# OPTML-Group/Unlearn-Saliency

Hardware: AMD Instinct MI355X
Metric: unlearn_steps_per_sec (ResNet-18/CIFAR-10 10%-forget, RL + SalUn mask, batch 256/GPU) (higher is better)
Workload: dtype f32

## Files before the change

### include/salun.h

```cpp
#ifndef SALUN_H
#define SALUN_H

#include <stddef.h>
#include <stdint.h>

#ifdef __cplusplus
extern "C" {
#endif

#define SALUN_OK 0
#define SALUN_EINVAL (-22)
#define SALUN_ENOSPC (-28)
#define SALUN_EIO (-5)

#define SALUN_MAX_THRESHOLDS 16

typedef void *salun_stream_t;

int salun_version(void);
const char *salun_strerror(int code);
const char *salun_arch(void);
int salun_clock_probe(unsigned long long *out , int samples, int spins, salun_stream_t stream);

int salun_saliency_accumulate(float *acc , const float *g ,
// ... 64 lines not shown
                     void *ws , size_t ws_bytes, salun_stream_t stream);

int salun_fim_square_accumulate(float *F , float *tmp , double n_data,
                                int64_t n, salun_stream_t stream);

int salun_conv2d_forward(const float *x , const float *w , const float *bias ,
                         float *y , int N, int C, int H, int W, int K, int R, int stride, int pad,
                         int P, int Q, salun_stream_t stream);
int salun_conv2d_forward_fused(const float *x , const float *w , const float *bias ,
                               const float *nbias , const float *addend ,
                               float *y , int N, int C, int H, int W, int K, int R, int stride, int pad,
                               int P, int Q, void *ws , size_t ws_bytes, salun_stream_t stream);
size_t salun_conv2d_data_workspace_bytes(int N, int outC, int outH, int outW, int R, int conv_stride);
int salun_conv2d_backward_data_ws(const float *dy , const float *w , const float *addend ,
                                  float *dx , int N, int C, int H, int W, int K, int R, int stride, int pad,
                                  int P, int Q, void *ws , size_t ws_bytes, salun_stream_t stream);
int salun_conv2d_backward_data(const float *dy , const float *w , float *dx , int N, int C,
                               int H, int W, int K, int R, int stride, int pad, int P, int Q,
                               salun_stream_t stream);
int salun_conv2d_backward_data_add(const float *dy , const float *w , const float *addend ,
                                   float *dx , int N, int C, int H, int W, int K, int R, int stride, int pad,
                                   int P, int Q, salun_stream_t stream);
size_t salun_channel_sum_workspace_bytes(int N, int K);
int salun_channel_sum(const float *dy , float *out , int N, int K, int HW, int accumulate,
                      void *ws , size_t ws_bytes, salun_stream_t stream);
size_t salun_conv2d_wgrad_workspace_bytes(int N, int C, int K, int R, int P, int Q);
int salun_conv2d_backward_weight(const float *x , const float *dy , float *dw , int N, int C,
                                 int H, int W, int K, int R, int stride, int pad, int P, int Q, int accumulate,
                                 void *ws , size_t ws_bytes, salun_stream_t stream);
#define SALUN_WGRAD_SHARED 1u
int salun_conv2d_backward_weight_ex(const float *x , const float *dy , float *dw , int N, int C,
                                    int H, int W, int K, int R, int stride, int pad, int P, int Q, int accumulate,
                                    unsigned flags, void *ws , size_t ws_bytes, salun_stream_t stream);
#define SALUN_ROUTE_FORWARD 0
#define SALUN_ROUTE_BACKWARD_DATA 1
#define SALUN_ROUTE_BACKWARD_WEIGHT 2
#define SALUN_ROUTE_EPI 2u
#define SALUN_ROUTE_W_UNALIGNED 4u
#define SALUN_ROUTE_OUT_UNALIGNED 8u
#define SALUN_ROUTE_IN_UNALIGNED 16u
int salun_conv2d_route(int direction, int N, int C, int H, int W, int K, int R, int stride, int pad, int P, int Q,
                       unsigned flags, size_t ws_bytes, char *buf, size_t buflen, int *nsplit );

size_t salun_conv3x3_pack_bytes(int K, int C, int dgrad);
#define SALUN_PACK_MAX_JOBS 32
typedef struct {
  const float *w;
  float *img_fwd;
  float *img_dgrad;
  int32_t K, C;
} salun_pack_job_t;
int salun_conv3x3_pack_weights(const salun_pack_job_t *jobs , int njobs, salun_stream_t stream);
int salun_conv3x3_packed(const float *x , const float *img , const float *bias ,
                         const float *nbias , const float *addend , float *y ,
                         int N, int Cred, int H, int W, int Kout, int cfg, salun_stream_t stream);

int salun_conv2d_bf16_supported(int C, int K, int R, int stride, int pad);
int salun_conv2d_bf16_pack_weights(const float *w , uint16_t *wp , int K, int C, int R,
                                   salun_stream_t stream);
#define SALUN_BF16_PACK_MAX_JOBS 64
typedef struct {
  const float *w;
  uint16_t *wp;
  int32_t K, C, R, transposed;
} salun_bf16_pack_job_t;
int salun_bf16_pack_weights_batch(const salun_bf16_pack_job_t *jobs, int n, salun_stream_t stream);
// ... 248 lines not shown
```

### unlearn_saliency_amd/_lib.py

```python
from __future__ import annotations

import ctypes
import os
import subprocess

_HERE = os.path.dirname(os.path.abspath(__file__))
LIB_PATH = os.environ.get("SALUN_LIB") or os.path.join(_HERE, "libsalun.so")
CSRC_DIR = os.path.join(_HERE, "csrc")

SALUN_OK = 0
SALUN_EINVAL = -22
SALUN_ENOSPC = -28
SALUN_EIO = -5
SALUN_MAX_THRESHOLDS = 16
SALUN_TOPK_FORCE_FULL_SCAN = 1
SALUN_TOPK_VALUES_ONLY = 2
SALUN_WGRAD_SHARED = 1

c_void_p, c_int, c_int64, c_uint64 = ctypes.c_void_p, ctypes.c_int, ctypes.c_int64, ctypes.c_uint64
c_double, c_size_t = ctypes.c_double, ctypes.c_size_t

class GemmSeg(ctypes.Structure):
    _fields_ = [("A", c_void_p), ("B", c_void_p), ("K", ctypes.c_int32), ("a_i", ctypes.c_int32),
                ("a_k", ctypes.c_int32), ("b_j", ctypes.c_int32), ("b_k", ctypes.c_int32)]
# ... 52 lines not shown
                                       c_double, c_double, c_double, c_double, c_double, c_double, c_int, c_int64,
                                       c_void_p]),
    "salun_adam_coefficients": (c_int, [c_void_p, c_double, c_double, c_double, c_void_p, c_void_p]),
    "salun_masked_adam_step_coef": (c_int, [c_void_p, c_void_p, c_void_p, c_void_p, c_void_p, c_void_p, c_double,
                                            c_double, c_void_p, c_double, c_double, c_double, c_double, c_int64,
                                            c_void_p]),
    "salun_adam_ema_step": (c_int, [c_void_p, c_void_p, c_void_p, c_void_p, c_void_p, c_void_p, c_void_p, c_double,
                                    c_double, c_double, c_double, c_double, c_double, c_double, c_double, c_int, c_int64,
                                    c_void_p]),
    "salun_adam_ema_step_coef": (c_int, [c_void_p, c_void_p, c_void_p, c_void_p, c_void_p, c_void_p, c_void_p, c_double,
                                         c_double, c_void_p, c_double, c_double, c_double, c_double, c_double, c_int64,
                                         c_void_p]),
    "salun_qsample": (c_int, [c_void_p, c_void_p, c_void_p, c_void_p, c_void_p, c_int64, c_void_p, c_int64, c_int64,
                              c_void_p]),
    "salun_sqerr_workspace_bytes": (c_size_t, [c_int64, c_int64]),
    "salun_sqerr_loss": (c_int, [c_void_p, c_void_p, c_int64, c_int64, c_double, c_void_p, c_void_p, c_void_p,
                                 c_void_p, c_size_t, c_void_p]),
    "salun_fim_square_accumulate": (c_int, [c_void_p, c_void_p, c_double, c_int64, c_void_p]),
    "salun_conv2d_forward": (c_int, [c_void_p, c_void_p, c_void_p, c_void_p] + [c_int] * 10 + [c_void_p]),
    "salun_conv2d_forward_fused": (c_int, [c_void_p] * 6 + [c_int] * 10 + [c_void_p, c_size_t, c_void_p]),
    "salun_conv2d_data_workspace_bytes": (c_size_t, [c_int] * 6),
    "salun_conv2d_backward_data_ws": (c_int, [c_void_p] * 4 + [c_int] * 10 + [c_void_p, c_size_t, c_void_p]),
    "salun_conv2d_backward_data": (c_int, [c_void_p, c_void_p, c_void_p] + [c_int] * 10 + [c_void_p]),
    "salun_channel_sum_workspace_bytes": (c_size_t, [c_int] * 2),
    "salun_channel_sum": (c_int, [c_void_p, c_void_p] + [c_int] * 4 + [c_void_p, c_size_t, c_void_p]),
    "salun_conv2d_wgrad_workspace_bytes": (c_size_t, [c_int] * 6),
    "salun_conv3x3_pack_bytes": (c_size_t, [c_int] * 3),
    "salun_conv3x3_pack_weights": (c_int, [c_void_p, c_int, c_void_p]),
    "salun_conv3x3_packed": (c_int, [c_void_p] * 6 + [c_int] * 6 + [c_void_p]),
    "salun_conv2d_backward_weight": (c_int, [c_void_p, c_void_p, c_void_p] + [c_int] * 11 + [c_void_p, c_size_t,
                                                                                          c_void_p]),
    "salun_conv2d_backward_weight_ex": (c_int, [c_void_p, c_void_p, c_void_p] + [c_int] * 11 + [ctypes.c_uint, c_void_p,
                                                                                                 c_size_t, c_void_p]),
    "salun_conv2d_route": (c_int, [c_int] * 11 + [ctypes.c_uint, c_size_t, ctypes.c_char_p, c_size_t,
                                   ctypes.POINTER(c_int)]),
    "salun_conv2d_bf16_supported": (c_int, [c_int] * 5),
    "salun_conv2d_bf16_pack_weights": (c_int, [c_void_p, c_void_p, c_int, c_int, c_int, c_void_p]),
    "salun_bf16_pack_weights_batch": (c_int, [c_void_p, c_int, c_void_p]),
    "salun_conv2d_bf16_data_workspace_bytes": (c_size_t, [c_int] * 8),
    "salun_conv2d_bf16_forward": (c_int, [c_void_p] * 6 + [c_int] * 8 + [c_void_p, c_size_t, c_void_p]),
    "salun_conv2d_bf16_backward_data": (c_int, [c_void_p] * 4 + [c_int] * 8 + [c_void_p, c_size_t, c_void_p]),
    "salun_conv2d_bf16_wgrad_workspace_bytes": (c_size_t, [c_int] * 8),
    "salun_conv2d_bf16_backward_weight": (c_int, [c_void_p] * 4 + [c_int] * 9 + [c_void_p, c_size_t, c_void_p]),
    "salun_colsum_bf16_workspace_bytes": (c_size_t, [c_int]),
    "salun_colsum_bf16": (c_int, [c_void_p, c_void_p, c_void_p, c_int64, c_int, c_int, c_int, c_void_p, c_size_t, c_void_p]),
    "salun_conv2d_bf16_backward_weight_ex": (c_int, [c_void_p] * 5 + [c_int] * 9 + [c_void_p, c_size_t, c_void_p]),
    "salun_gn_bf16_workspace_bytes": (c_size_t, [c_int] * 4),
    "salun_gn_bf16_forward": (c_int, [c_void_p] * 6 + [c_int] * 4 + [c_double, c_int, c_void_p, c_size_t, c_void_p]),
    "salun_gn_bf16_backward": (c_int, [c_void_p] * 8 + [c_int] * 6 + [c_void_p, c_size_t, c_void_p]),
    "salun_attn_supported": (c_int, [c_int]),
    "salun_attn_forward": (c_int, [c_void_p] * 5 + [c_int] * 5 + [ctypes.c_longlong, c_int] * 4 + [c_double, c_void_p]),
    "salun_attn_backward": (c_int, [c_void_p] * 10 + [c_int] * 5 + [ctypes.c_longlong, c_int] * 5 + [c_double, c_void_p]),
    "salun_ln_bf16_workspace_bytes": (c_size_t, [c_int64, c_int]),
    "salun_ln_bf16_forward": (c_int, [c_void_p] * 5 + [c_int64, c_int, c_double, c_void_p]),
    "salun_ln_bf16_backward": (c_int, [c_void_p] * 7 + [c_int64, c_int, c_int, c_void_p, c_size_t, c_void_p]),
    "salun_geglu_bf16_forward": (c_int, [c_void_p, c_void_p, c_int64, c_int, c_void_p]),
    "salun_geglu_bf16_backward": (c_int, [c_void_p, c_void_p, c_void_p, c_int64, c_int, c_void_p]),
    "salun_bn_workspace_bytes": (c_size_t, [c_int]),
    "salun_bn_forward": (c_int, [c_void_p] * 10 + [c_int] * 4 + [c_double, c_double, c_int, c_void_p, c_size_t, c_void_p]),
    "salun_bn_backward": (c_int, [c_void_p] * 12 + [c_int] * 5 + [c_void_p, c_size_t, c_void_p]),
    "salun_conv2d_backward_data_add": (c_int, [c_void_p] * 4 + [c_int] * 10 + [c_void_p]),
    "salun_gn_workspace_bytes": (c_size_t, [c_int, c_int]),
    "salun_gn_forward": (c_int, [c_void_p] * 6 + [c_int] * 4 + [c_double, c_int, c_void_p]),
    "salun_gn_backward": (c_int, [c_void_p] * 11 + [c_int] * 5 + [c_void_p, c_size_t, c_void_p]),
    "salun_gn_backward_fused": (c_int, [c_void_p] * 15 + [c_int] * 5 + [c_void_p, c_size_t, c_void_p]),
    "salun_param_diff": (c_int, [c_void_p, c_void_p, c_void_p, c_int64, c_void_p]),
# ... 102 lines not shown
```

### unlearn_saliency_amd/csrc/salun_conv.hip

```cpp
#include "salun_common.h"
#include "salun_conv_plan.h"
#include <mutex>
#include <type_traits>
#include <unordered_set>

int salun_ring_wgrad_launch(const float *x, const float *dy, float *part, int N, int C, int H, int W, int K, int nsplit,
                            int nchunks, hipStream_t st);

namespace {

typedef float f32x16 __attribute__((ext_vector_type(16)));

struct PatchPos {
  int goff;
  int loff;
  int valid;
};

__device__ __forceinline__ void tile_origin(int tile, int NI, int TP, int tiles_per_img, int &n0, int &p0) {
  if (NI > 1) { n0 = tile * NI; p0 = 0; }
  else { n0 = tile / tiles_per_img; p0 = (tile - n0 * tiles_per_img) * TP; }
}

struct LanePix {
// ... 392 lines not shown
#pragma unroll
      for (int t = 0; t < KT; ++t) a_cur[t] = a_nxt[t];
    }
  }

  const int n_out = n0 + lp.ni;
  const int h_out = (p0 + lp.p) * g.os + g.ph, w_out = lp.q * g.os + g.pw;
  if (n_out < g.N) {
#pragma unroll
    for (int t = 0; t < KT; ++t) {
      const int kbase = k0 + (wk * KT + t) * 32 + 4 * hi;
      const size_t obase = (((size_t)n_out * g.yC + kbase) * g.yH + h_out) * g.yW + w_out;
      const size_t kstride = (size_t)g.yH * g.yW;
      float bv[16];
      const int klast = g.yC - 1 - kbase;
      if (g.bias) {
#pragma unroll
        for (int v = 0; v < 16; ++v)
          bv[v] = g.bias[obase + (long long)acc_row_clamped(v, klast, kbase) * (long long)kstride];
      }
#pragma unroll
      for (int v = 0; v < 16; ++v) {
        const int kr = acc_row(v);
        if (kbase + kr < g.yC) {
          float o = acc[t][v];
          if (g.bias) o += bv[v];
          g.y[obase + kr * kstride] = o;
        }
      }
    }
  }
}

template <int R, int PAD, int KT, int WP, int WK>
__global__ __launch_bounds__(256, 2) void conv_dgrad_s2(const float *__restrict__ dy, const float *__restrict__ w,
                                                     const float *__restrict__ addend, float *__restrict__ dx, int N,
                                                     int K, int P, int Q, int C, int H, int W, int NI, int TP,
                                                     int IH_t, int IW_t, int logQ) {
  constexpr int RS = R * R;
  constexpr int KB = WK * KT * 32;
  constexpr int WROW = CC * RS + 1;
  constexpr int DMIN = (R == 1) ? 0 : (PAD == 1 ? 0 : -1);
  constexpr int FP = (R == 1) ? 1 : 2;
  constexpr int NCLS = (R == 1) ? 1 : 4;
  extern __shared__ __attribute__((aligned(16))) float lds[];
  const int PSZ = NI * IH_t * IW_t;
  const int ch_stride = PSZ | 1;
  float *patch = lds;
  float *wl = lds + CC * ch_stride;

  const int tid = threadIdx.x, lane = tid & 63, wave = tid >> 6;
  const int lo = lane & 31, hi = lane >> 5;
  const int wp = wave % WP, wk = wave / WP;
  const int c0out = blockIdx.y * KB;
  const int tiles_per_img = (NI > 1) ? 1 : P / TP;
  const int tile = blockIdx.x;
  int n0, p0;
  if (NI > 1) { n0 = tile * NI; p0 = 0; }
  else { n0 = tile / tiles_per_img; p0 = (tile - n0 * tiles_per_img) * TP; }
  const LanePix lp = lane_pixel(wp * 32 + lo, Q, logQ, TP, IH_t, IW_t, 1);

  const int planePQ = P * Q;
  int goff = 0;
  bool valid = false;
  if (tid < PSZ) {
    const int ni = tid / (IH_t * IW_t);
    const int rem = tid - ni * (IH_t * IW_t);
    const int ih = rem / IW_t, iw = rem - ih * IW_t;
    const int n = n0 + ni;
    const int pp = p0 + DMIN + ih, qq = DMIN + iw;
    valid = (n < N) && pp >= 0 && pp < P && qq >= 0 && qq < Q;
// ... 72 lines not shown
#pragma unroll
        for (int rs = 0; rs < RS; ++rs) av[t][rs] = wb0[t * 32 * WROW + cc * RS + rs];
    };
    float b_cur[FP * FP], a_cur[KT][RS], b_nxt[FP * FP], a_nxt[KT][RS];
    operands(0, b_cur, a_cur);
#pragma unroll
    for (int step = 0; step < NSTEP; ++step) {
      if (step + 1 < NSTEP) operands(step + 1, b_nxt, a_nxt);
      __builtin_amdgcn_sched_barrier(0);
#pragma unroll
      for (int r = 0; r < R; ++r)
#pragma unroll
        for (int s2 = 0; s2 < R; ++s2) {
          const int ph = (R == 1) ? 0 : ((r - PAD) & 1), pw = (R == 1) ? 0 : ((s2 - PAD) & 1);
          const int di = (R == 1) ? 0 : ((ph + PAD - r) / 2 - DMIN), dj = (R == 1) ? 0 : ((pw + PAD - s2) / 2 - DMIN);
          const int cls = (R == 1) ? 0 : (ph * 2 + pw);
#pragma unroll
          for (int t = 0; t < KT; ++t)
            acc[cls][t] = __builtin_amdgcn_mfma_f32_32x32x2f32(a_cur[t][r * R + s2], b_cur[di * FP + dj], acc[cls][t],
                                                               0, 0, 0);
        }
      __builtin_amdgcn_sched_barrier(0);
      if (step + 1 < NSTEP) {
#pragma unroll
        for (int i = 0; i < FP * FP; ++i) b_cur[i] = b_nxt[i];
#pragma unroll
        for (int t = 0; t < KT; ++t)
#pragma unroll
          for (int rs = 0; rs < RS; ++rs) a_cur[t][rs] = a_nxt[t][rs];
      }
    }
  }

  const int n_out = n0 + lp.ni;
  const int a_out = p0 + lp.p;
  if (n_out < N) {
#pragma unroll
    for (int t = 0; t < KT; ++t) {
      const int cbase = c0out + (wk * KT + t) * 32 + 4 * hi;
      const size_t obase = (((size_t)n_out * C + cbase) * H + 2 * a_out) * W + 2 * lp.q;
      const size_t cstride = (size_t)H * W;
#pragma unroll
      for (int vb = 0; vb < 16; vb += 8) {
        float2 ad[8][2];
        const int clast = C - 1 - cbase;
        if (addend) {
#pragma unroll
          for (int u = 0; u < 8; ++u) {
            const int v = vb + u, cr = acc_row_clamped(v, clast, cbase);
#pragma unroll
            for (int ph = 0; ph < 2; ++ph)
              ad[u][ph] = *reinterpret_cast<const float2 *>(addend + obase + (long long)cr * (long long)cstride + ph * W);
          }
        }
#pragma unroll
        for (int u = 0; u < 8; ++u) {
          const int v = vb + u, cr = acc_row(v);
          if (cbase + cr < C) {
#pragma unroll
            for (int ph = 0; ph < 2; ++ph) {
              float2 o;
              if (R == 1) {
                o.x = (ph == 0) ? acc[0][t][v] : 0.f;
                o.y = 0.f;
              } else {
                o.x = acc[ph * 2 + 0][t][v];
                o.y = acc[ph * 2 + 1][t][v];
              }
              if (addend) {
                o.x += ad[u][ph].x;
                o.y += ad[u][ph].y;
              }
              *reinterpret_cast<float2 *>(dx + obase + cr * cstride + ph * W) = o;
// ... 821 lines not shown
      if (!p.fast) {
        launch_one_igemm<R, STRIDE, KT, WP, WK, DGRAD, false, 1, false, false>(p, a, st);
      } else if (p.S > 1) {
        if constexpr (CAN_SPLIT) launch_one_igemm<R, STRIDE, KT, WP, WK, DGRAD, true, 1, true, false>(p, a, st);
      } else if (p.epi) {
        if constexpr (CAN_EPI) launch_one_igemm<R, STRIDE, KT, WP, WK, DGRAD, true, 1, false, true>(p, a, st);
      } else {
        launch_one_igemm<R, STRIDE, KT, WP, WK, DGRAD, true, 1, false, false>(p, a, st);
      }
    });
  }
  SALUN_LAUNCH_CHECK();
  if (p.S > 1) {
    hipLaunchKernelGGL(conv_split_finish, dim3((unsigned)((p.out_elems / 4 + 255) / 256)), dim3(256), 0, st, a.part, p.S,
                       p.out_elems, DGRAD ? nullptr : a.bias, a.nbias, a.addend, DGRAD ? a.bias : nullptr, a.y, a.yC,
                       a.yH * a.yW);
    SALUN_LAUNCH_CHECK();
  }
  return SALUN_OK;
}

inline int launch_data(const DataPlan &p, const DataArgs &a, hipStream_t st) {
  if (p.dgrad) return p.R == 3 ? launch_data<3, 1, true>(p, a, st) : launch_data<1, 1, true>(p, a, st);
  if (p.R == 3) return p.stride == 1 ? launch_data<3, 1, false>(p, a, st) : launch_data<3, 2, false>(p, a, st);
  return p.stride == 1 ? launch_data<1, 1, false>(p, a, st) : launch_data<1, 2, false>(p, a, st);
}

template <int R, int PAD, int KT, int WP, int WK>
void launch_one_dgrad_s2(const Dgrad2Plan &p, const float *dy, const float *w, const float *addend, float *dx, int N,
                         int C, int H, int W, int K, int P, int Q, hipStream_t st) {
  const TileGeom &g = p.t.g;
  allow_lds(conv_dgrad_s2<R, PAD, KT, WP, WK>, p.lds_bytes);
  hipLaunchKernelGGL((conv_dgrad_s2<R, PAD, KT, WP, WK>), dim3(g.ntiles, C / p.t.kb()), dim3(256), p.lds_bytes, st, dy, w,
                     addend, dx, N, K, P, Q, C, H, W, g.NI, g.TP, g.IH_t, g.IW_t, g.logQ);
}

template <int RH, int RW, int KT, int WP, int WK, int MAXPOS>
void launch_one_dgrad_tap(const TapClass &c, const TapArgs &a, hipStream_t st) {
  allow_lds(conv_dgrad_tap<RH, RW, KT, WP, WK, MAXPOS>, c.lds_bytes);
  hipLaunchKernelGGL((conv_dgrad_tap<RH, RW, KT, WP, WK, MAXPOS>), dim3(c.t.g.ntiles, (a.yC + c.t.kb() - 1) / c.t.kb()),
                     dim3(256), c.lds_bytes, st, a);
}

inline int launch_dgrad_s2(const Dgrad2Plan &p, const float *dy, const float *w, const float *addend, float *dx, int N,
                           int C, int H, int W, int K, int P, int Q, hipStream_t st) {
  if (p.merged) {
    with_tile(p.t, [&](auto kt, auto wp, auto wk) {
      constexpr int KT = decltype(kt)::value, WP = decltype(wp)::value, WK = decltype(wk)::value;
      if constexpr (KT <= 2) {
        if (p.R == 1) launch_one_dgrad_s2<1, 0, KT, WP, WK>(p, dy, w, addend, dx, N, C, H, W, K, P, Q, st);
        else if (p.pad == 1) launch_one_dgrad_s2<3, 1, KT, WP, WK>(p, dy, w, addend, dx, N, C, H, W, K, P, Q, st);
        else launch_one_dgrad_s2<3, 0, KT, WP, WK>(p, dy, w, addend, dx, N, C, H, W, K, P, Q, st);
      }
    });
    SALUN_LAUNCH_CHECK();
    return SALUN_OK;
  }
  TapArgs a{};
  a.x = dy; a.w = w; a.bias = addend; a.y = dx;
  a.N = N; a.xC = K; a.xH = P; a.xW = Q; a.yC = C; a.yH = H; a.yW = W;
  a.wC = C; a.wK = K; a.Rfull = p.R;
  a.subH = H / 2; a.subW = W / 2; a.os = 2; a.ts = 2;
  if (p.any_empty) {
    const size_t bytes = sizeof(float) * (size_t)N * C * H * W;
    if (!addend) {
      if (hipMemsetAsync(dx, 0, bytes, st) != hipSuccess) return SALUN_EIO;
    } else if (addend != dx) {
// ... 225 lines not shown
  if (!dy || !out || !ws || N < 1 || K < 1 || HW < 1) return SALUN_EINVAL;
  const int S = channel_sum_splits(N, K);
  if (ws_bytes < sizeof(float) * (size_t)K * S) return SALUN_ENOSPC;
  if (K > 65535 * 16) return SALUN_EINVAL;
  hipStream_t st = salun_hip_stream(stream);
  float *part = static_cast<float *>(ws);
  hipLaunchKernelGGL(k_channel_sum_partial, dim3(K, S), dim3(256), 0, st, dy, part, N, K, HW, S);
  SALUN_LAUNCH_CHECK();
  hipLaunchKernelGGL(k_channel_sum_final, dim3((K + 255) / 256), dim3(256), 0, st, part, out, K, S, accumulate);
  SALUN_LAUNCH_CHECK();
  return SALUN_OK;
}

SALUN_EXPORT int salun_conv2d_backward_weight(const float *x, const float *dy, float *dw, int N, int C, int H, int W,
                                              int K, int R, int stride, int pad, int P, int Q, int accumulate,
                                              void *ws, size_t ws_bytes, salun_stream_t stream) {
  return salun_conv2d_backward_weight_ex(x, dy, dw, N, C, H, W, K, R, stride, pad, P, Q, accumulate, 0, ws, ws_bytes, stream);
}

SALUN_EXPORT int salun_conv2d_backward_weight_ex(const float *x, const float *dy, float *dw, int N, int C, int H, int W,
                                                 int K, int R, int stride, int pad, int P, int Q, int accumulate,
                                                 unsigned flags, void *ws, size_t ws_bytes, salun_stream_t stream) {
  if (!x || !dy || !dw || !ws) return SALUN_EINVAL;
  const WgradPlan p = plan_wgrad(N, C, H, W, K, R, stride, pad, P, Q, (flags & SALUN_WGRAD_SHARED) != 0,
                                 salun_aligned16(x) && salun_aligned16(dy), ws_bytes);
  if (p.rc != SALUN_OK) return p.rc;
  hipStream_t st = salun_hip_stream(stream);
  const WgradArgs a{x, dy, static_cast<float *>(ws), N, C, H, W, K, P, Q, pad};
  const int rc = launch_wgrad(p, a, st);
  if (rc != SALUN_OK) return rc;
  launch_wgrad_reduce(a.part, dw, (int64_t)K * C * R * R, p.nsplit, accumulate, K * C, R * R, st);
  SALUN_LAUNCH_CHECK();
  return SALUN_OK;
}

SALUN_EXPORT int salun_conv2d_route(int direction, int N, int C, int H, int W, int K, int R, int stride, int pad, int P,
                                    int Q, unsigned flags, size_t ws_bytes, char *buf, size_t buflen, int *nsplit) {
  if (!buf || buflen < 1) return SALUN_EINVAL;
  buf[0] = 0;
  if (nsplit) *nsplit = 0;
  const bool w_al16 = !(flags & SALUN_ROUTE_W_UNALIGNED), out_al16 = !(flags & SALUN_ROUTE_OUT_UNALIGNED);
  const bool in_al16 = !(flags & SALUN_ROUTE_IN_UNALIGNED);
  int rc = SALUN_EINVAL, len = 0;
  if (direction == SALUN_ROUTE_FORWARD) {
    const DataPlan p = plan_data(N, C, K, P, Q, R, stride, false, C, (flags & SALUN_ROUTE_EPI) != 0, w_al16, out_al16,
                                 ws_bytes);
    if ((rc = p.rc) == SALUN_OK) len = data_label(buf, buflen, p);
  } else if (direction == SALUN_ROUTE_BACKWARD_DATA && (P < 1 || Q < 1)) {
  } else if (direction == SALUN_ROUTE_BACKWARD_DATA && stride == 1) {
    const DataPlan p = plan_data(N, K, C, H, W, R, 1, true, C, false, w_al16, out_al16, ws_bytes);
    if ((rc = p.rc) == SALUN_OK) len = data_label(buf, buflen, p);
  } else if (direction == SALUN_ROUTE_BACKWARD_DATA && stride == 2) {
    const Dgrad2Plan p = plan_dgrad_s2(N, C, H, W, K, R, pad, P, Q, w_al16, out_al16);
    if ((rc = p.rc) == SALUN_OK) len = dgrad2_label(buf, buflen, p);
  } else if (direction == SALUN_ROUTE_BACKWARD_WEIGHT) {
    const WgradPlan p = plan_wgrad(N, C, H, W, K, R, stride, pad, P, Q, (flags & SALUN_WGRAD_SHARED) != 0, in_al16,
                                   ws_bytes);
    if ((rc = p.rc) == SALUN_OK) {
      len = wgrad_label(buf, buflen, p);
      if (nsplit) *nsplit = p.nsplit;
    }
  }
  if (rc == SALUN_OK && (len < 0 || (size_t)len >= buflen)) { buf[0] = 0; return SALUN_ENOSPC; }
  return rc;
}
```

### unlearn_saliency_amd/csrc/salun_conv_plan.h

```cpp
#pragma once
#include <cstddef>
#include <cstdio>
#include "../../include/salun.h"

bool salun_ring_wgrad_fits(int N, int C, int H, int W, int K, int nchunks, bool in_al16);

namespace {

constexpr int CC = 8;
constexpr int igemm_chunk(int R, int stride) { return (R == 1 && stride == 1) ? 32 : CC; }

constexpr int tap_chunk(int taps) { return taps == 1 ? 32 : taps == 2 ? 16 : 8; }

struct TileGeom {
  int NI, TP, IH_t, IW_t, logQ;
  int ntiles;
  bool ok;
  int psz() const { return NI * IH_t * IW_t; }
};

inline int ilog2(int v) {
  int l = 0;
  while ((1 << l) < v) ++l;
  return l;
// ... 295 lines not shown
  if (!shifts) return p;
  p.lds_bytes = sizeof(float) * 2 * ((size_t)64 * (g.psz() | 1) + (size_t)64 * (pixc + 1) + 256);
  if ((size_t)g.NI * C * H * W >= (1u << 30) || (size_t)g.NI * K * P * Q >= (1u << 30)) return p;
  if (p.lds_bytes > 160 * 1024) return p;
  p.rc = SALUN_OK;
  p.fullC = C % 64 == 0;
  if (R == 3 && stride == 1 && pad == 1 && P == H && Q == W && !shared &&
      salun_ring_wgrad_fits(N, C, H, W, K, g.ntiles, in_al16)) {
    p.route = WG_RING;
    return p;
  }
  if (R == 3 && pad == 1 && p.fullC && W % 4 == 0 && Q * stride == W && P * stride == H && in_al16 &&
      (size_t)g.NI * C * H * W < (1u << 30)) {
    const int F4C = g.NI * g.IH_t * (W / 4);
    const int nit = (F4C % 4 == 0) ? F4C / 4 : 0;
    if (stride == 1 ? (nit == 5 || nit == 6 || nit == 8) : (nit == 9 || nit == 10)) {
      p.route = WG_V;
      p.nit = nit;
    }
  }
  return p;
}

inline int wgrad_label(char *buf, size_t n, const WgradPlan &p) {
  switch (p.route) {
    case WG_1X1: return snprintf(buf, n, "wgrad_1x1<%d>", p.stride);
    case WG_SMALLC: return snprintf(buf, n, "wgrad_smallc<%d,%d>", p.R, p.stride);
    case WG_RING: return snprintf(buf, n, "wgrad_ring<W%d>", p.W);
    case WG_V: return snprintf(buf, n, "wgrad_v<%d,%d>", p.stride, p.nit);
    default: return snprintf(buf, n, "wgrad<%d,%d,%s>", p.R, p.stride, p.fullC ? "true" : "false");
  }
}

}
```

### unlearn_saliency_amd/ops.py

```python
from __future__ import annotations

import ctypes
from typing import Optional, Sequence

import torch

from .fastfn import FastFunction

from . import _lib, ringpack, weightimg
from ._lib import c_double, c_int, c_int64, c_size_t, c_uint64, c_void_p, check
from .streams import _stream, _stream_handle


def _dev(t: Optional[torch.Tensor], dtype: torch.dtype, name: str, allow_none: bool = False) -> c_void_p:
    if t is None:
        if allow_none:
            return c_void_p(None)
        raise ValueError(f"{name} must not be None")
    if not t.is_cuda:
        raise RuntimeError(f"{name}: the SalUn HIP kernels need a device tensor (got {t.device}); no CPU fallback")
    if t.dtype != dtype:
        raise TypeError(f"{name}: expected {dtype}, got {t.dtype}")
    if not t.is_contiguous():
        raise ValueError(f"{name} must be contiguous")
# ... 384 lines not shown
        return None
    check(rc, "salun_conv2d_backward_data")
    return dx


WGRAD_KERNEL = [None]


def conv2d_backward_weight(x: torch.Tensor, dy: torch.Tensor, w_shape, stride: int, pad: int,
                           out: Optional[torch.Tensor] = None, accumulate: bool = False,
                           shared: bool = False, stream: Optional[torch.cuda.Stream] = None) -> Optional[torch.Tensor]:
    N, C, H, W = x.shape
    K, _, R, _ = w_shape
    P, Q = dy.shape[2], dy.shape[3]
    L = _lib.lib()
    nbytes = L.salun_conv2d_wgrad_workspace_bytes(N, C, K, R, P, Q)
    if nbytes == 0:
        return None
    ws = workspace(nbytes, x.device, stream=stream)
    dw = out if out is not None else torch.empty(tuple(w_shape), dtype=torch.float32, device=x.device)
    rc = L.salun_conv2d_backward_weight_ex(_dev(x, torch.float32, "x"), _dev(dy, torch.float32, "dy"),
                                           _dev(dw, torch.float32, "dw"), N, C, H, W, K, R, stride, pad, P, Q,
                                           int(bool(accumulate and out is not None)),
                                           _lib.SALUN_WGRAD_SHARED if (shared if WGRAD_KERNEL[0] is None
                                                                       else WGRAD_KERNEL[0] == "shared") else 0,
                                           c_void_p(ws.data_ptr()), c_size_t(ws.numel()),
                                           c_void_p(_stream_handle() if stream is None else stream.cuda_stream))
    if rc == _lib.SALUN_EINVAL:
        return None
    check(rc, "salun_conv2d_backward_weight")
    return dw


def conv3x3_pack(w: torch.Tensor, dgrad: bool, out: Optional[torch.Tensor] = None) -> Optional[torch.Tensor]:
    K, C = w.shape[0], w.shape[1]
    L = _lib.lib()
    nbytes = int(L.salun_conv3x3_pack_bytes(K, C, int(dgrad)))
    if nbytes == 0 or tuple(w.shape[2:]) != (3, 3):
        return None
    img = out if out is not None and out.numel() * 4 == nbytes else torch.empty(nbytes // 4, dtype=torch.float32,
                                                                                device=w.device)
    _dev(w, torch.float32, "w")
    job = _lib.PackJob(w.data_ptr(), None if dgrad else img.data_ptr(), img.data_ptr() if dgrad else None, K, C)
    check(L.salun_conv3x3_pack_weights(ctypes.cast(ctypes.pointer(job), c_void_p), 1, _stream()),
          "salun_conv3x3_pack_weights")
    return img


def conv3x3_packed(x: torch.Tensor, img: torch.Tensor, Kout: int, bias: Optional[torch.Tensor] = None,
                   nbias: Optional[torch.Tensor] = None, addend: Optional[torch.Tensor] = None,
                   out: Optional[torch.Tensor] = None, cfg: int = 0) -> Optional[torch.Tensor]:
    N, Cred, H, W = x.shape
    y = out if out is not None else torch.empty((N, Kout, H, W), dtype=torch.float32, device=x.device)
    rc = _lib.lib().salun_conv3x3_packed(_dev(x, torch.float32, "x"), c_void_p(img.data_ptr()),
                                         _dev(bias, torch.float32, "bias", True),
                                         _dev(nbias, torch.float32, "nbias", True),
                                         _dev(addend, torch.float32, "addend", True), c_void_p(y.data_ptr()),
                                         N, Cred, H, W, Kout, int(cfg), _stream())
    if rc == _lib.SALUN_EINVAL:
        return None
    check(rc, "salun_conv3x3_packed")
    return y


def channel_sum(dy: torch.Tensor, out: Optional[torch.Tensor] = None, accumulate: bool = False) -> torch.Tensor:
    N, K = dy.shape[0], dy.shape[1]
# ... 527 lines not shown
```

### unlearn_saliency_amd/resblock.py

```python
from __future__ import annotations

import torch

from .fastfn import FastFunction
import torch.nn as nn

import os

from . import dist as sdist
from . import draws, gradsink, ops, wgrad_side

FWD_SHORTCUT_BESIDE = os.environ.get("SALUN_FWD_SHORTCUT_BESIDE", "1") != "0"


def _bn_args(bn: nn.BatchNorm2d):
    return bn.running_mean, bn.running_var, bn.training, bn.momentum, bn.eps


class _BasicBlockFn(FastFunction):
    @staticmethod
    def forward(ctx, x, blk, w1, g1, b1, w2, g2, b2, wd, gd, bd):
        s = blk.conv1.stride[0]
        N, C, H, W = x.shape
        P, Q = (H + 2 - 3) // s + 1, (W + 2 - 3) // s + 1
        training = blk.bn1.training
        cd = md = idd = None
        fork = None
        if wd is not None:
            def shortcut():
                cd_ = ops.conv2d_forward(x, wd, None, s, 0, P, Q)
                return (cd_,) + tuple(ops.bn_forward(cd_, None, gd, bd, *_bn_args(blk.downsample[1]), False,
                                                     blk.downsample[1].num_batches_tracked))
            if (FWD_SHORTCUT_BESIDE and wgrad_side.OVERLAP and x.is_cuda
                    and not torch.cuda.is_current_stream_capturing()):
                main, fork = torch.cuda.current_stream(x.device), wgrad_side.stream(x.device)
                fork.wait_stream(main)
                with torch.cuda.stream(fork):
                    cd, skip, md, idd = shortcut()
                x.record_stream(fork)
        c1 = ops.conv2d_forward(x, w1, None, s, 1, P, Q)
        y1, m1, i1 = ops.bn_forward(c1, None, g1, b1, *_bn_args(blk.bn1), True, blk.bn1.num_batches_tracked)
        c2 = ops.conv2d_forward(y1, w2, None, 1, 1, P, Q)
        if wd is None:
            skip = x
        elif fork is None:
            cd, skip, md, idd = shortcut()
        else:
            main.wait_stream(fork)
            for t in (cd, skip, md, idd):
                if t is not None:
                    t.record_stream(main)
        out, m2, i2 = ops.bn_forward(c2, skip, g2, b2, *_bn_args(blk.bn2), True, blk.bn2.num_batches_tracked)
        ctx.save_for_backward(x, c1, y1, c2, out, cd, w1, g1, b1, w2, g2, b2, wd, gd, bd, m1, i1, m2, i2, md, idd)
        ctx.cfg = (s, training)
        return out

    @staticmethod
    def backward(ctx, dout):
        x, c1, y1, c2, out, cd, w1, g1, b1, w2, g2, b2, wd, gd, bd, m1, i1, m2, i2, md, idd = ctx.saved_tensors
        s, training = ctx.cfg
        dout = dout.contiguous()
        grads = {}

        def bn_bwd(dy, y, xin, g, b, m, i, relu, want_dres):
            gw, gb = gradsink.sink(g), gradsink.sink(b)
            if gw is None or gb is None:
                gw = gb = None
            dx, dres, dg, db = ops.bn_backward(dy, y, xin, g, m, i, training, relu, want_dres, gw, gb)
            if gw is not None:
                gradsink.arrived(g)
                gradsink.arrived(b)
                dg = db = None
            return dx, dres, dg, db

        dev = dout.device
        overlap = wgrad_side.OVERLAP

        def wgrad(xin, dy, w, stride, pad):
            dst = gradsink.sink(w)
            if overlap:
                dw = wgrad_side.beside(dev, (xin, dy), lambda side: ops.conv2d_backward_weight(
                    xin, dy, w.shape, stride, pad, out=dst, accumulate=True, shared=True, stream=side), alloc=dst is None)
            else:
                dw = ops.conv2d_backward_weight(xin, dy, w.shape, stride, pad, out=dst, accumulate=True)
            if dst is not None:
                gradsink.arrived(w)
                return None
            return dw

        dc2, dskip, dg2, db2 = bn_bwd(dout, out, c2, g2, b2, m2, i2, True, True)
        dwd = dgd = dbd = None
        dxd = dskip
        if wd is not None:
            dcd, _, dgd, dbd = bn_bwd(dskip, None, cd, gd, bd, md, idd, False, False)
            dwd = wgrad(x, dcd, wd, s, 0)
            dxd = ops.conv2d_backward_data(dcd, wd, x.shape, s, 0) if ctx.needs_input_grad[0] else None
        dw2 = wgrad(y1, dc2, w2, 1, 1)
        dy1 = ops.conv2d_backward_data(dc2, w2, y1.shape, 1, 1)
        dc1, _, dg1, db1 = bn_bwd(dy1, y1, c1, g1, b1, m1, i1, True, False)
        dw1 = wgrad(x, dc1, w1, s, 1)
        dx = ops.conv2d_backward_data(dc1, w1, x.shape, s, 1, addend=dxd) if ctx.needs_input_grad[0] else None
        if overlap and not all(g is None for g in (dw1, dw2, dwd)):
            torch.cuda.current_stream(dev).wait_stream(wgrad_side.stream(dev))
            wgrad_side.release_held(dev)
        return dx, None, dw1, dg1, db1, dw2, dg2, db2, dwd, dgd, dbd


def _probe(blk, shape, device) -> bool:
    N, C, H, W = shape
    s = blk.conv1.stride[0]
    P, Q = (H + 2 - 3) // s + 1, (W + 2 - 3) // s + 1
    K = blk.conv1.out_channels
    if (P * Q) % 4 or (H * W) % 4:
        return False
    e = lambda *sh: torch.empty(sh, dtype=torch.float32, device=device)
    x, y1, dy = e(N, C, H, W), e(N, K, P, Q), e(N, K, P, Q)
    convs = [(x, blk.conv1.weight, s, 1), (y1, blk.conv2.weight, 1, 1)]
    if blk.downsample is not None:
        convs.append((x, blk.downsample[0].weight, s, 0))
    for xin, w, st, pad in convs:
        if ops.conv2d_forward(xin, w, None, st, pad, P, Q) is None:
            return False
        if ops.conv2d_backward_data(dy, w, xin.shape, st, pad, addend=xin) is None:
            return False
        if ops.conv2d_backward_weight(xin, dy, w.shape, st, pad) is None:
            return False
    return True


def _structure_ok(blk) -> bool:
    convs = [blk.conv1, blk.conv2] + ([blk.downsample[0]] if blk.downsample is not None else [])
    bns = [blk.bn1, blk.bn2] + ([blk.downsample[1]] if blk.downsample is not None else [])
    if any(type(b) is not nn.BatchNorm2d or not b.affine or not b.track_running_stats or b.momentum is None
           for b in bns):
        return False
    if any(c.bias is not None or c.groups != 1 or c.dilation != (1, 1) or c.weight.dtype != torch.float32
           for c in convs):
        return False
    if len({b.training for b in bns}) != 1:
        return False
    c1, c2 = blk.conv1, blk.conv2
    ok = (c1.kernel_size == (3, 3) and c1.padding == (1, 1) and c1.stride[0] == c1.stride[1] and c1.stride[0] in (1, 2)
          and c2.kernel_size == (3, 3) and c2.padding == (1, 1) and c2.stride == (1, 1))
    if blk.downsample is not None:
        d = blk.downsample[0]
        ok = ok and d.kernel_size == (1, 1) and d.padding == (0, 0) and d.stride == c1.stride
    else:
        ok = ok and c1.stride == (1, 1) and c1.in_channels == c1.out_channels
    return ok


def fused_basic_block(blk, x: torch.Tensor):
    if not (x.is_cuda and x.dtype == torch.float32 and x.dim() == 4) or torch.is_autocast_enabled():
        return None
    cache = blk.__dict__.setdefault("_fused_shapes", {})
    key = (tuple(x.shape), x.device)
    ok = cache.get(key)
    if ok is None:
        with torch.no_grad():
            ok = cache[key] = _structure_ok(blk) and _probe(blk, tuple(x.shape), x.device)
# ... 179 lines not shown
```

Baseline: 118.1.

## Fuse strided block's 3x3 and 1x1 projection data-gradients into one kernel

Adds a paired variant of the stride-2 dgrad kernel. It runs the 1x1 projection shortcut's data-gradient GEMM on the same output tile after the 3x3 conv1 dgrad and sums the two in registers before writing dx. The separate shortcut dgrad launch is dropped, along with the full-size intermediate dxd tensor and its read back as an addend. This costs extra register pressure and LDS reuse in the kernel, plus a per-shape probe cache in Python.

Measured after the change: 118.3 (median of 2 runs). No clear change (+0.1%).

```diff
diff --git a/include/salun.h b/include/salun.h
--- a/include/salun.h
+++ b/include/salun.h
@@ -120,6 +120,10 @@
 int salun_conv2d_backward_weight_ex(const float *x , const float *dy , float *dw , int N, int C,
                                     int H, int W, int K, int R, int stride, int pad, int P, int Q, int accumulate,
                                     unsigned flags, void *ws , size_t ws_bytes, salun_stream_t stream);
+int salun_conv2d_backward_data_pair(const float *dy , const float *w , const float *dy2 ,
+                                    const float *w2 , const float *addend , float *dx ,
+                                    int N, int C, int H, int W, int K, int K2, int pad, int P, int Q,
+                                    salun_stream_t stream);
 #define SALUN_ROUTE_FORWARD 0
 #define SALUN_ROUTE_BACKWARD_DATA 1
 #define SALUN_ROUTE_BACKWARD_WEIGHT 2
diff --git a/unlearn_saliency_amd/_lib.py b/unlearn_saliency_amd/_lib.py
--- a/unlearn_saliency_amd/_lib.py
+++ b/unlearn_saliency_amd/_lib.py
@@ -108,6 +108,7 @@
                                                                                           c_void_p]),
     "salun_conv2d_backward_weight_ex": (c_int, [c_void_p, c_void_p, c_void_p] + [c_int] * 11 + [ctypes.c_uint, c_void_p,
                                                                                                  c_size_t, c_void_p]),
+    "salun_conv2d_backward_data_pair": (c_int, [c_void_p] * 6 + [c_int] * 9 + [c_void_p]),
     "salun_conv2d_route": (c_int, [c_int] * 11 + [ctypes.c_uint, c_size_t, ctypes.c_char_p, c_size_t,
                                    ctypes.POINTER(c_int)]),
     "salun_conv2d_bf16_supported": (c_int, [c_int] * 5),
diff --git a/unlearn_saliency_amd/csrc/salun_conv.hip b/unlearn_saliency_amd/csrc/salun_conv.hip
--- a/unlearn_saliency_amd/csrc/salun_conv.hip
+++ b/unlearn_saliency_amd/csrc/salun_conv.hip
@@ -448,11 +448,13 @@
   }
 }
 
-template <int R, int PAD, int KT, int WP, int WK>
+template <int R, int PAD, int KT, int WP, int WK, bool PAIR = false>
 __global__ __launch_bounds__(256, 2) void conv_dgrad_s2(const float *__restrict__ dy, const float *__restrict__ w,
+                                                     const float *__restrict__ dy2, const float *__restrict__ w2,
                                                      const float *__restrict__ addend, float *__restrict__ dx, int N,
-                                                     int K, int P, int Q, int C, int H, int W, int NI, int TP,
+                                                     int K, int K2, int P, int Q, int C, int H, int W, int NI, int TP,
                                                      int IH_t, int IW_t, int logQ) {
+  static_assert(!PAIR || (R == 3 && PAD == 1), "the pair is conv1 of a strided block with its projection");
   constexpr int RS = R * R;
   constexpr int KB = WK * KT * 32;
   constexpr int WROW = CC * RS + 1;
@@ -591,13 +593,81 @@
     }
   }
 
-  const int n_out = n0 + lp.ni;
-  const int a_out = p0 + lp.p;
+  LanePix lpe = lp;
+  int hie = hi, wke = wk;
+  if constexpr (PAIR) {
+    constexpr int W2ROW = CC + 1;
+    constexpr int N2F4 = CC * KB / 4;
+    static_assert(N2F4 <= 256 && KB * W2ROW <= KB * WROW, "one 16-byte load per thread; inside the 3x3 slab's region");
+    int tid2 = threadIdx.x;
+    asm volatile("" : "+v"(tid2));
+    const int lo2 = tid2 & 31, hi2 = (tid2 >> 5) & 1, wave2 = tid2 >> 6;
+    const LanePix lp2 = lane_pixel((wave2 % WP) * 32 + lo2, Q, logQ, TP, IH_t, IW_t, 1);
+    const int goff2 = goff + (goff / planePQ / K) * (K2 - K) * planePQ;
+    const int row2 = tid2 / (KB / 4), q42 = tid2 - row2 * (KB / 4);
+    auto load_chunk2 = [&](int k0) {
+      if (valid) {
+        const float *src = dy2 + goff2 + k0 * planePQ;
+#pragma unroll
+        for (int c = 0; c < CC; ++c) preg[c] = src[c * planePQ];
+      } else {
+#pragma unroll
+        for (int c = 0; c < CC; ++c) preg[c] = 0.f;
+      }
+      if (N2F4 == 256 || tid2 < N2F4)
+        wreg4[0] = *reinterpret_cast<const float4 *>(w2 + (size_t)(k0 + row2) * C + c0out + 4 * q42);
+    };
+    auto store_chunk2 = [&]() {
+      if (tid2 < PSZ) {
+#pragma unroll
+        for (int c = 0; c < CC; ++c) patch[c * ch_stride + tid2] = preg[c];
+      }
+      if (N2F4 == 256 || tid2 < N2F4) {
+        wl[(4 * q42 + 0) * W2ROW + row2] = wreg4[0].x;
+        wl[(4 * q42 + 1) * W2ROW + row2] = wreg4[0].y;
+        wl[(4 * q42 + 2) * W2ROW + row2] = wreg4[0].z;
+        wl[(4 * q42 + 3) * W2ROW + row2] = wreg4[0].w;
+      }
+    };
+    f32x16 acc2[KT];
+#pragma unroll
+    for (int t = 0; t < KT; ++t)
+#pragma unroll
+      for (int v = 0; v < 16; ++v) acc2[t][v] = 0.f;
+    load_chunk2(0);
+    for (int k0 = 0; k0 < K2; k0 += CC) {
+      __syncthreads();
+      store_chunk2();
+      __syncthreads();
+      if (k0 + CC < K2) load_chunk2(k0 + CC);
+      const float *pb0 = patch + hi2 * ch_stride + lp2.off;
+      const float *wb0 = wl + ((wave2 / WP) * KT * 32 + lo2) * W2ROW + hi2;
+#pragma unroll
+      for (int step = 0; step < CC / 2; ++step) {
+        const float b = pb0[2 * step * ch_stride];
+#pragma unroll
+        for (int t = 0; t < KT; ++t)
+          acc2[t] = __builtin_amdgcn_mfma_f32_32x32x2f32(wb0[t * 32 * W2ROW + 2 * step], b, acc2[t], 0, 0, 0);
+      }
+    }
+#pragma unroll
+    for (int cl = 0; cl < NCLS; ++cl)
+#pragma unroll
+      for (int t = 0; t < KT; ++t)
+#pragma unroll
+        for (int v = 0; v < 16; ++v) acc[cl][t][v] += (cl == 0) ? acc2[t][v] : 0.f;
+    lpe = lp2;
+    hie = hi2;
+    wke = wave2 / WP;
+  }
+
+  const int n_out = n0 + lpe.ni;
+  const int a_out = p0 + lpe.p;
   if (n_out < N) {
 #pragma unroll
     for (int t = 0; t < KT; ++t) {
-      const int cbase = c0out + (wk * KT + t) * 32 + 4 * hi;
-      const size_t obase = (((size_t)n_out * C + cbase) * H + 2 * a_out) * W + 2 * lp.q;
+      const int cbase = c0out + (wke * KT + t) * 32 + 4 * hie;
+      const size_t obase = (((size_t)n_out * C + cbase) * H + 2 * a_out) * W + 2 * lpe.q;
       const size_t cstride = (size_t)H * W;
 #pragma unroll
       for (int vb = 0; vb < 16; vb += 8) {
@@ -1485,7 +1555,24 @@
   const TileGeom &g = p.t.g;
   allow_lds(conv_dgrad_s2<R, PAD, KT, WP, WK>, p.lds_bytes);
   hipLaunchKernelGGL((conv_dgrad_s2<R, PAD, KT, WP, WK>), dim3(g.ntiles, C / p.t.kb()), dim3(256), p.lds_bytes, st, dy, w,
-                     addend, dx, N, K, P, Q, C, H, W, g.NI, g.TP, g.IH_t, g.IW_t, g.logQ);
+                     nullptr, nullptr, addend, dx, N, K, 0, P, Q, C, H, W, g.NI, g.TP, g.IH_t, g.IW_t, g.logQ);
+}
+
+inline int launch_dgrad_pair(const DgradPairPlan &pp, const float *dy, const float *w, const float *dy2, const float *w2,
+                             const float *addend, float *dx, int N, int C, int H, int W, int K, int K2, int P, int Q,
+                             hipStream_t st) {
+  const Tile &t = pp.d.t;
+  const TileGeom &g = t.g;
+  with_tile(t, [&](auto kt, auto wp, auto wk) {
+    constexpr int KT = decltype(kt)::value, WP = decltype(wp)::value, WK = decltype(wk)::value;
+    if constexpr (KT <= 2) {
+      allow_lds(conv_dgrad_s2<3, 1, KT, WP, WK, true>, pp.lds_bytes);
+      hipLaunchKernelGGL((conv_dgrad_s2<3, 1, KT, WP, WK, true>), dim3(g.ntiles, C / t.kb()), dim3(256), pp.lds_bytes, st,
+                         dy, w, dy2, w2, addend, dx, N, K, K2, P, Q, C, H, W, g.NI, g.TP, g.IH_t, g.IW_t, g.logQ);
+    }
+  });
+  SALUN_LAUNCH_CHECK();
+  return SALUN_OK;
 }
 
 template <int RH, int RW, int KT, int WP, int WK, int MAXPOS>
@@ -1777,6 +1864,16 @@
   launch_wgrad_reduce(a.part, dw, (int64_t)K * C * R * R, p.nsplit, accumulate, K * C, R * R, st);
   SALUN_LAUNCH_CHECK();
   return SALUN_OK;
+}
+
+SALUN_EXPORT int salun_conv2d_backward_data_pair(const float *dy, const float *w, const float *dy2, const float *w2,
+                                                 const float *addend, float *dx, int N, int C, int H, int W, int K,
+                                                 int K2, int pad, int P, int Q, salun_stream_t stream) {
+  if (!dy || !w || !dy2 || !w2 || !dx) return SALUN_EINVAL;
+  const bool out_al16 = salun_aligned16(dx) && (!addend || salun_aligned16(addend));
+  const DgradPairPlan pp = plan_dgrad_pair(N, C, H, W, K, K2, pad, P, Q, salun_aligned16(w), salun_aligned16(w2), out_al16);
+  if (pp.rc != SALUN_OK) return pp.rc;
+  return launch_dgrad_pair(pp, dy, w, dy2, w2, addend, dx, N, C, H, W, K, K2, P, Q, salun_hip_stream(stream));
 }
 
 SALUN_EXPORT int salun_conv2d_route(int direction, int N, int C, int H, int W, int K, int R, int stride, int pad, int P,
diff --git a/unlearn_saliency_amd/csrc/salun_conv_plan.h b/unlearn_saliency_amd/csrc/salun_conv_plan.h
--- a/unlearn_saliency_amd/csrc/salun_conv_plan.h
+++ b/unlearn_saliency_amd/csrc/salun_conv_plan.h
@@ -351,4 +351,23 @@
   }
 }
 
-}
+struct DgradPairPlan {
+  int rc;
+  Dgrad2Plan d;
+  size_t lds_bytes;
+};
+
+inline DgradPairPlan plan_dgrad_pair(int N, int C, int H, int W, int K, int K2, int pad, int P, int Q, bool w_al16,
+                                     bool w2_al16, bool out_al16) {
+  DgradPairPlan pp{};
+  pp.rc = SALUN_EINVAL;
+  if (pad != 1 || K2 < CC || K2 % CC != 0 || !w2_al16 || C % 4 != 0) return pp;
+  pp.d = plan_dgrad_s2(N, C, H, W, K, 3, 1, P, Q, w_al16, out_al16);
+  if (pp.d.rc != SALUN_OK || !pp.d.merged) return pp;
+  if ((size_t)N * K2 * P * Q >= ((size_t)1 << 31) || (size_t)N * K * P * Q >= ((size_t)1 << 31)) return pp;
+  pp.lds_bytes = pp.d.lds_bytes;
+  pp.rc = SALUN_OK;
+  return pp;
+}
+
+}
diff --git a/unlearn_saliency_amd/ops.py b/unlearn_saliency_amd/ops.py
--- a/unlearn_saliency_amd/ops.py
+++ b/unlearn_saliency_amd/ops.py
@@ -440,6 +440,27 @@
     return dw
 
 
+def conv2d_backward_data_pair(dy: torch.Tensor, w: torch.Tensor, dy2: torch.Tensor, w2: torch.Tensor, x_shape,
+                              addend: Optional[torch.Tensor] = None) -> Optional[torch.Tensor]:
+    N, C, H, W = x_shape
+    K, K2 = w.shape[0], w2.shape[0]
+    P, Q = dy.shape[2], dy.shape[3]
+    if (tuple(w.shape[1:]) != (C, 3, 3) or tuple(w2.shape[1:]) != (C, 1, 1) or tuple(dy.shape) != (N, K, P, Q)
+            or tuple(dy2.shape) != (N, K2, P, Q)):
+        return None
+    if addend is not None and tuple(addend.shape) != (N, C, H, W):
+        raise ValueError(f"addend must be {(N, C, H, W)}, got {tuple(addend.shape)}")
+    dx = torch.empty((N, C, H, W), dtype=torch.float32, device=dy.device)
+    rc = _lib.lib().salun_conv2d_backward_data_pair(_dev(dy, torch.float32, "dy"), _dev(w, torch.float32, "w"),
+                                                    _dev(dy2, torch.float32, "dy2"), _dev(w2, torch.float32, "w2"),
+                                                    _dev(addend, torch.float32, "addend", True),
+                                                    c_void_p(dx.data_ptr()), N, C, H, W, K, K2, 1, P, Q, _stream())
+    if rc == _lib.SALUN_EINVAL:
+        return None
+    check(rc, "salun_conv2d_backward_data_pair")
+    return dx
+
+
 def conv3x3_pack(w: torch.Tensor, dgrad: bool, out: Optional[torch.Tensor] = None) -> Optional[torch.Tensor]:
     K, C = w.shape[0], w.shape[1]
     L = _lib.lib()
diff --git a/unlearn_saliency_amd/resblock.py b/unlearn_saliency_amd/resblock.py
--- a/unlearn_saliency_amd/resblock.py
+++ b/unlearn_saliency_amd/resblock.py
@@ -11,6 +11,7 @@
 from . import draws, gradsink, ops, wgrad_side
 
 FWD_SHORTCUT_BESIDE = os.environ.get("SALUN_FWD_SHORTCUT_BESIDE", "1") != "0"
+STRIDED_PAIR = os.environ.get("SALUN_STRIDED_PAIR", "1") != "0"
 
 
 def _bn_args(bn: nn.BatchNorm2d):
@@ -52,13 +53,13 @@
                     t.record_stream(main)
         out, m2, i2 = ops.bn_forward(c2, skip, g2, b2, *_bn_args(blk.bn2), True, blk.bn2.num_batches_tracked)
         ctx.save_for_backward(x, c1, y1, c2, out, cd, w1, g1, b1, w2, g2, b2, wd, gd, bd, m1, i1, m2, i2, md, idd)
-        ctx.cfg = (s, training)
+        ctx.cfg = (s, training, wd is not None and STRIDED_PAIR and _pair_ok(blk, tuple(x.shape), x.device))
         return out
 
     @staticmethod
     def backward(ctx, dout):
         x, c1, y1, c2, out, cd, w1, g1, b1, w2, g2, b2, wd, gd, bd, m1, i1, m2, i2, md, idd = ctx.saved_tensors
-        s, training = ctx.cfg
+        s, training, pair = ctx.cfg
         dout = dout.contiguous()
         grads = {}
 
@@ -91,15 +92,23 @@
         dc2, dskip, dg2, db2 = bn_bwd(dout, out, c2, g2, b2, m2, i2, True, True)
         dwd = dgd = dbd = None
         dxd = dskip
+        dcd = None
         if wd is not None:
             dcd, _, dgd, dbd = bn_bwd(dskip, None, cd, gd, bd, md, idd, False, False)
             dwd = wgrad(x, dcd, wd, s, 0)
-            dxd = ops.conv2d_backward_data(dcd, wd, x.shape, s, 0) if ctx.needs_input_grad[0] else None
+            dxd = ops.conv2d_backward_data(dcd, wd, x.shape, s, 0) if ctx.needs_input_grad[0] and not pair else None
         dw2 = wgrad(y1, dc2, w2, 1, 1)
         dy1 = ops.conv2d_backward_data(dc2, w2, y1.shape, 1, 1)
         dc1, _, dg1, db1 = bn_bwd(dy1, y1, c1, g1, b1, m1, i1, True, False)
         dw1 = wgrad(x, dc1, w1, s, 1)
-        dx = ops.conv2d_backward_data(dc1, w1, x.shape, s, 1, addend=dxd) if ctx.needs_input_grad[0] else None
+        if not ctx.needs_input_grad[0]:
+            dx = None
+        elif pair:
+            dx = ops.conv2d_backward_data_pair(dc1, w1, dcd, wd, x.shape)
+            if dx is None:
+                raise RuntimeError("strided-block pair refused a shape its probe accepted")
+        else:
+            dx = ops.conv2d_backward_data(dc1, w1, x.shape, s, 1, addend=dxd)
         if overlap and not all(g is None for g in (dw1, dw2, dwd)):
             torch.cuda.current_stream(dev).wait_stream(wgrad_side.stream(dev))
             wgrad_side.release_held(dev)
@@ -126,6 +135,26 @@
         if ops.conv2d_backward_weight(xin, dy, w.shape, st, pad) is None:
             return False
     return True
+
+
+def _pair_ok(blk, shape, device) -> bool:
+    cache = blk.__dict__.setdefault("_pair_shapes", {})
+    key = (shape, device)
+    ok = cache.get(key)
+    if ok is None:
+        N, C, H, W = shape
+        s = blk.conv1.stride[0]
+        P, Q = (H + 2 - 3) // s + 1, (W + 2 - 3) // s + 1
+        K = blk.conv1.out_channels
+        w1, wd = blk.conv1.weight, blk.downsample[0].weight
+        ok = s == 2 and wd.shape[0] == K
+        if ok:
+            with torch.no_grad():
+                e = lambda *sh: torch.empty(sh, dtype=torch.float32, device=device)
+                dy = e(N, K, P, Q)
+                ok = ops.conv2d_backward_data_pair(dy, w1, dy, wd, shape) is not None
+        cache[key] = ok
+    return ok
 
 
 def _structure_ok(blk) -> bool:
```
